# chaofengc/FeMaSR

Hardware: AMD Instinct MI355X
Metric: SR output megapixels/sec at x4 (128->512) (higher is better)
Workload: dtype f32 (1x1 convs / nn.Linear: every fp32 operand split EXACTLY into three bf16 terms, six partial products, fp32 accumulation on the bf16 matrix pipe - closer to fp64 than the fp32 fmaf chain, bit-identical to the CPU oracle)

## Files before the change

### femasr_amd/_lib.py

```python
import ctypes
import os

_HERE = os.path.dirname(os.path.abspath(__file__))
SO_PATH = os.path.join(_HERE, 'csrc', 'libfemasr_hip.so')

c_int, c_i64, c_f32 = ctypes.c_int, ctypes.c_int64, ctypes.c_float
vp, szt = ctypes.c_void_p, ctypes.c_size_t


class FemasrError(RuntimeError):
    pass


MAX_CODEBOOKS = 3


class Config(ctypes.Structure):
    _fields_ = ([(n, ctypes.c_int32) for n in ('in_channel', 'gt_resolution', 'lq_stage', 'scale_factor', 'use_quantize',
                                               'use_residual', 'n_codebooks')] +
                [(n, ctypes.c_int32 * MAX_CODEBOOKS) for n in ('codebook_scale', 'n_e', 'e_dim')] +
                [('device', ctypes.c_int32)])


class ConvArgs(ctypes.Structure):
    _fields_ = [
        ('in_', vp), ('B', ctypes.c_int32), ('H', ctypes.c_int32), ('W', ctypes.c_int32), ('Cin', ctypes.c_int32),
        ('w', vp), ('bias', vp),
        ('Cout', ctypes.c_int32), ('ksz', ctypes.c_int32), ('stride', ctypes.c_int32), ('pad', ctypes.c_int32),
        ('up2', ctypes.c_int32), ('prologue', ctypes.c_int32),
        ('pro_a', vp), ('pro_b', vp), ('pro_c', vp),
        ('act', ctypes.c_int32),
        ('res1', vp), ('res2', vp), ('out', vp),
        ('Ho', ctypes.c_int32), ('Wo', ctypes.c_int32),
        ('w_bf16x3', vp), ('gn_part', vp), ('w_up2', vp), ('w_wino', vp), ('fast_act', ctypes.c_int32), ('in_add', vp), ('w_bf16s', vp),
        ('w_f16', vp),
    ]


ABI_VERSION = 107
PRO_NONE, PRO_GN_SILU, PRO_LN = 0, 1, 2
ACT_NONE, ACT_GELU, ACT_RELU = 0, 1, 2

SIGNATURES = {
    'femasr_last_error': (ctypes.c_char_p, []),
    'femasr_version': (c_int, []),
    'femasr_create': (c_int, [ctypes.POINTER(Config), ctypes.POINTER(vp)]),
    'femasr_destroy': (None, [vp]),
    'femasr_num_weights': (c_int, [vp]),
    'femasr_weight_info': (c_int, [vp, c_int, ctypes.POINTER(ctypes.c_char_p), ctypes.POINTER(c_i64 * 4), ctypes.POINTER(c_int)]),
# ... 87 lines not shown
    'femasr_dihedral_expand': (c_int, [vp, vp, c_int, c_int, c_int, c_int, vp, vp]),
    'femasr_dihedral_expand_u8': (c_int, [vp, vp, c_int, c_int, c_int, vp, vp]),
    'femasr_dihedral_merge': (c_int, [vp, vp, vp, c_int, c_int, c_int, c_int, vp]),
    'femasr_dihedral_merge_u8': (c_int, [vp, vp, vp, c_int, c_int, c_int, vp]),
    'femasr_png_filter_rgb8': (c_int, [vp, vp, c_int, c_int, c_int, c_int, vp]),
    'femasr_clock_probe': (c_int, [vp, c_int, vp]),
    'femasr_clock_probe_entries': (c_int, []),
}
DEBUG_SIGNATURES = {
    'femasr_debug_set_wino_limits': (c_int, [vp, c_int, c_int]),
    'femasr_debug_mfma_bf16': (c_int, [vp, vp, vp, vp, c_int, vp]),
    'femasr_gemm_force_config': (c_int, [c_int]),
    'femasr_conv_small_launch_blocks': (c_int, [c_int]),
    'femasr_debug_conv_variant_name': (c_int, [ctypes.POINTER(ConvArgs), ctypes.c_char_p, c_int]),
    'femasr_debug_weight_image_bytes': (c_int, [vp, c_int, ctypes.POINTER(szt)]),
}

_lib = None


def load():
    global _lib
    if _lib is not None:
        return _lib
    if not os.path.exists(SO_PATH):
        raise FemasrError(
            f'{SO_PATH} not found: the HIP extension is not built. Run `python femasr_amd/csrc/build.py` '
            '(needs hipcc; cross-compiles gfx950 without a GPU). There is no CPU fallback.')
    lib = ctypes.CDLL(SO_PATH)
    lib.femasr_version.restype = c_int
    if lib.femasr_version() != ABI_VERSION:
# ... 19 lines not shown
```

### femasr_amd/csrc/kernels_gemm_bf16.hip

```cpp
#include "conv_common.h"
#include "detmath.h"
#include <stdlib.h>

typedef float f32x16 __attribute__((ext_vector_type(16)));
typedef __bf16 bf16x8 __attribute__((ext_vector_type(8)));
typedef __bf16 bf16x2_t __attribute__((ext_vector_type(2)));
typedef float f32x2_t __attribute__((ext_vector_type(2)));

namespace {

struct GemmSParams {
    const float *A;
    const uint4 *W;
    const float *bias, *res1, *res2;
    float *out;
    int M, N, K, MB, NB, NT32;
    int imH, imW, Cin, tapmul;
    int imHo, imWo, stride;
};

__device__ float g_gs_zero_page[64];

constexpr int GS_A_HALF = 3 * 2 * 128;
constexpr int GS_A_BYTES = 2 * GS_A_HALF * 16;
constexpr int GS_W_STAGE = 4 * 3 * 64;
constexpr int GS_W_STAGES = 4;
constexpr int GS_LDS_BYTES = GS_A_BYTES + GS_W_STAGES * GS_W_STAGE * 16;
static_assert(4 * TSCRATCH * 4 <= GS_LDS_BYTES, "epilogue scratch overlays the main-loop buffers");

__device__ __forceinline__ unsigned cvt_pk_bf16(float a, float b)
{
    const bf16x2_t r = __builtin_convertvector(f32x2_t{a, b}, bf16x2_t);
    return __builtin_bit_cast(unsigned, r);
// ... 186 lines not shown
                d1[k] = *reinterpret_cast<const f32x4_t *>(ra + o);
                if (NRES >= 2) d2[k] = *reinterpret_cast<const f32x4_t *>(rb + o);
            }
        };
        if (vec) {
#pragma unroll
            for (int j = 0; j < 2; ++j) {
                const int col = n0 + (wn * 2 + j) * 32 + 4 * tq;
                bpre[j] = *reinterpret_cast<const f32x4_t *>(p.bias + (col < p.N ? col : 0));
            }
        }
        fetch_res(0, r1[0], r2[0]);
        asm volatile("s_waitcnt lgkmcnt(0)" ::: "memory");
        __builtin_amdgcn_s_barrier();
        asm volatile("" ::: "memory");
#pragma unroll
        for (int tl = 0; tl < 4; ++tl) {
            const int i = tl >> 1, j = tl & 1;
            const int rbase = m0 + (wm * 2 + i) * 32, cbase = n0 + (wn * 2 + j) * 32;
            if (vec) {
                const int col = cbase + 4 * tq;
                const bool cok = col < p.N;
                if (tl + 1 < 4) fetch_res(tl + 1, r1[(tl + 1) & 1], r2[(tl + 1) & 1]);
#pragma unroll
                for (int r = 0; r < 16; ++r) T[((r & 3) + 8 * (r >> 2) + 4 * h) * TPITCH + c31] = hi[i][j][r] + lo[i][j][r];
                const f32x4_t b4 = bpre[j];
#pragma unroll
                for (int k = 0; k < 4; ++k) {
                    const f32x4_t a4 = *reinterpret_cast<const f32x4_t *>(T + (trow + 8 * k) * TPITCH + 4 * tq);
                    float v[4] = {a4[0] + b4[0], a4[1] + b4[1], a4[2] + b4[2], a4[3] + b4[3]};
                    if (ACT == FEMASR_ACT_GELU) {
                        const det_f32x2 g0 = det_gelu2(det_f32x2{v[0], v[1]}), g1 = det_gelu2(det_f32x2{v[2], v[3]});
                        v[0] = g0[0]; v[1] = g0[1]; v[2] = g1[0]; v[3] = g1[1];
                    }
#pragma unroll
                    for (int e = 0; e < 4; ++e) {
                        if (NRES >= 1) v[e] = v[e] + r1[tl & 1][k][e];
                        if (NRES >= 2) v[e] = v[e] + r2[tl & 1][k][e];
                    }
                    const int row = rbase + trow + 8 * k;
                    if (cok && row < p.M) *reinterpret_cast<f32x4_t *>(p.out + (size_t)row * p.N + col) = f32x4_t{v[0], v[1], v[2], v[3]};
                }
            } else {
                const int col = cbase + c31;
#pragma unroll
                for (int r = 0; r < 16; ++r) {
                    const int row = rbase + (r & 3) + 8 * (r >> 2) + 4 * h;
                    if (row < p.M && col < p.N) {
                        const size_t o = (size_t)row * p.N + col;
                        float v = (hi[i][j][r] + lo[i][j][r]) + p.bias[col];
                        if (ACT == FEMASR_ACT_GELU) v = det_gelu(v);
                        if (NRES >= 1) v = v + ra[o];
                        if (NRES >= 2) v = v + rb[o];
                        p.out[o] = v;
                    }
                }
// ... 132 lines not shown
{
    FEMASR_REQUIRE(a && a->in && w_bf16s && femasr_gemm_bf16s_shape_ok(a), "gemm_bf16s: layer is neither a 1x1 / linear layer nor a 3x3 pad-1 conv of stride 1 or 2 with Cin %% 64 == 0");
    FEMASR_REQUIRE(a->bias && a->out, "gemm_bf16s: bias/out must be set");
    FEMASR_REQUIRE(a->act == FEMASR_ACT_NONE || a->act == FEMASR_ACT_GELU, "gemm_bf16s: bad activation %d", a->act);
    const bool conv = a->ksz == 3;
    const int Ho = conv ? (a->H - 1) / a->stride + 1 : a->H, Wo = conv ? (a->W - 1) / a->stride + 1 : a->W;
    const long long M = (long long)a->B * Ho * Wo;
    FEMASR_REQUIRE(a->Ho == Ho && a->Wo == Wo, "gemm_bf16s: Ho/Wo mismatch");
    FEMASR_REQUIRE(M > 0 && M < (1ll << 31) - 256, "gemm_bf16s: bad row count");
    GemmSParams p{};
    p.A = a->in; p.W = (const uint4 *)w_bf16s; p.bias = a->bias; p.res1 = a->res1; p.res2 = a->res2; p.out = a->out;
    p.M = (int)M; p.N = a->Cout; p.K = conv ? 9 * a->Cin : a->Cin;
    p.imH = a->H; p.imW = a->W; p.imHo = Ho; p.imWo = Wo; p.stride = a->stride; p.Cin = a->Cin; p.tapmul = ((1 << 20) + (a->Cin >> 5) - 1) / (a->Cin >> 5);
    p.NT32 = (p.N + 31) / 32;
    p.MB = (p.M + 127) / 128; p.NB = (p.N + 127) / 128;
    const int vi = femasr_gemm_bf16s_pick_variant(a);
    GSVariant &v = g_gsv[vi];
    FEMASR_CHECK(femasr_allow_dynamic_lds((const void *)v.kern, &v.attr_devs, GS_LDS_BYTES));
    hipLaunchKernelGGL(v.kern, dim3((unsigned)(p.MB * p.NB)), dim3(256), (size_t)GS_LDS_BYTES, s, p);
    FEMASR_CHECK_HIP(hipGetLastError());
    if (variant_out) *variant_out = vi;
    if (flops_out) *flops_out = 2.0 * (double)M * (double)a->Cout * (double)p.K;
    return FEMASR_OK;
}
```

### femasr_amd/csrc/kernels_misc.hip

```cpp
#include "common.h"
#include "detmath.h"
#include <stdlib.h>
#include <string.h>
#include <type_traits>

namespace {

__device__ __forceinline__ float4 ld4(const float *p) { return *reinterpret_cast<const float4 *>(p); }

__device__ __forceinline__ int xcd_remap_misc(int bid, int nblk)
{
    const int q = nblk >> 3, r = nblk & 7, xcd = bid & 7, within = bid >> 3;
    return (xcd < r ? xcd * (q + 1) : r * (q + 1) + (xcd - r) * q) + within;
}

__global__ void pad_nchw_to_nhwc_kernel(const float *__restrict__ in, int B, int C, int H, int W, int Hp, int Wp,
                                        float *__restrict__ out, size_t total)
{
    for (size_t i = blockIdx.x * (size_t)blockDim.x + threadIdx.x; i < total; i += (size_t)gridDim.x * blockDim.x) {
        const int c = (int)(i % C);
        size_t r = i / C;
        const int x = (int)(r % Wp);
        r /= Wp;
        const int y = (int)(r % Hp);
// ... 287 lines not shown
    q = __builtin_fmaf(d, d, q);
    const float var = wave_tree_sum(q) * (1.0f / 256.0f);
    const float rstd = 1.0f / sqrtf(var + eps);
    const float4 g = ld4(gamma + lane * 4), b = ld4(beta + lane * 4);
    float4 o;
    o.x = __builtin_fmaf((v.x - mean) * rstd, g.x, b.x);
    o.y = __builtin_fmaf((v.y - mean) * rstd, g.y, b.y);
    o.z = __builtin_fmaf((v.z - mean) * rstd, g.z, b.z);
    o.w = __builtin_fmaf((v.w - mean) * rstd, g.w, b.w);
    *reinterpret_cast<float4 *>(y + row * 256 + lane * 4) = o;
}

constexpr int ATT_HD = 32, ATT_N = 64;
typedef float att_f32x16 __attribute__((ext_vector_type(16)));

template <int UNITS>
__global__ __launch_bounds__(64, 2) void window_attention_reg_kernel(const float *__restrict__ qkv, int B, int H, int W, int C,
                                                                     int heads, int shift, const float *__restrict__ table,
                                                                     float *__restrict__ out, int total)
{
    __shared__ float Ts[UNITS][232];
    const int lane = threadIdx.x, c = lane & 31, hf = lane >> 5;
    const int nwx = W >> 3, nwy = H >> 3;
    struct Unit { int h, wx, wy, n; };
    auto unit_of = [&](int bid) {
        Unit g;
        g.h = bid % heads;
        bid /= heads;
        g.wx = bid % nwx;
        bid /= nwx;
        g.wy = bid % nwy;
        g.n = bid / nwy;
        return g;
    };
    Unit gs[UNITS];
    bool has[UNITS];
#pragma unroll
    for (int u = 0; u < UNITS; ++u) {
        const int bid = (int)blockIdx.x * UNITS + u;
        has[u] = bid < total;
        gs[u] = unit_of(has[u] ? bid : total - 1);
        for (int i = lane; i < 225; i += 64) Ts[u][i] = table[i * heads + gs[u].h];
    }
    const float scale = 0.17677669529663687f;
    auto rowtok = [&](const Unit &g, int iy) { int y = g.wy * 8 + iy + shift; if (y >= H) y -= H; return y * W; };
    auto coltok = [&](const Unit &g, int ix) { int x = g.wx * 8 + ix + shift; if (x >= W) x -= W; return x; };
    auto qb = [&](const Unit &g) { return qkv + (size_t)g.n * H * W * 3 * C + g.h * ATT_HD; };

    float ak[2][16], bq[2][16];
    auto load_qk = [&](const Unit &g) {
        const float *qbase = qb(g);
#pragma unroll
        for (int tI = 0; tI < 2; ++tI) {
            const int w = 32 * tI + c;
            const unsigned tok = (unsigned)(rowtok(g, w >> 3) + coltok(g, w & 7));
            const float *kp = qbase + tok * (unsigned)(3 * C) + C, *qp = qbase + tok * (unsigned)(3 * C);
#pragma unroll
            for (int d4 = 0; d4 < 8; ++d4) {
                const float4 kv = ld4(kp + 4 * d4), qv = ld4(qp + 4 * d4);
                ak[tI][2 * d4] = hf ? kv.y : kv.x;
                ak[tI][2 * d4 + 1] = hf ? kv.w : kv.z;
                bq[tI][2 * d4] = (hf ? qv.y : qv.x) * scale;
                bq[tI][2 * d4 + 1] = (hf ? qv.w : qv.z) * scale;
            }
        }
    };
    load_qk(gs[0]);
#pragma unroll
    for (int u = 0; u < UNITS; ++u) {
        if (!has[u]) break;
        const Unit g = gs[u];
        const float *qbase = qb(g);
        float *obase = out + (size_t)g.n * H * W * C + g.h * ATT_HD;
        const bool masked = shift > 0 && (g.wy == nwy - 1 || g.wx == nwx - 1);
        att_f32x16 sc[2][2];
#pragma unroll
        for (int tj = 0; tj < 2; ++tj)
#pragma unroll
            for (int ti = 0; ti < 2; ++ti)
#pragma unroll
                for (int r = 0; r < 16; ++r) sc[tj][ti][r] = 0.f;
#pragma unroll
        for (int st = 0; st < 16; ++st)
#pragma unroll
            for (int tj = 0; tj < 2; ++tj)
#pragma unroll
                for (int ti = 0; ti < 2; ++ti) sc[tj][ti] = __builtin_amdgcn_mfma_f32_32x32x2f32(ak[tj][st], bq[ti][st], sc[tj][ti], 0, 0, 0);

        float vf[2][16];
        {
            const float *vb = qbase + 2 * C + c;
            unsigned cto[4];
#pragma unroll
            for (int e = 0; e < 4; ++e) cto[e] = (unsigned)coltok(g, e + 4 * hf) * (unsigned)(3 * C);
#pragma unroll
            for (int tj = 0; tj < 2; ++tj)
#pragma unroll
                for (int r = 0; r < 16; ++r) {
                    const unsigned ro = (unsigned)__builtin_amdgcn_readfirstlane(rowtok(g, (r >> 2) + 4 * tj)) * (unsigned)(3 * C);
                    vf[tj][r] = vb[ro + cto[r & 3]];
                }
        }
        if (u + 1 < UNITS && has[u + 1 < UNITS ? u + 1 : u]) load_qk(gs[u + 1 < UNITS ? u + 1 : u]);
#pragma unroll
        for (int ti = 0; ti < 2; ++ti) {
// ... 517 lines not shown
                       gamma, beta, eps, y);
    FEMASR_CHECK_HIP(hipGetLastError());
    return FEMASR_OK;
}

int femasr_window_attention(void *stream, const float *qkv, int B, int H, int W, int C, int heads, int shift,
                            const float *table, float *out)
{
    FEMASR_REQUIRE(qkv && table && out && B > 0, "window_attention: bad args");
    FEMASR_REQUIRE(H % 8 == 0 && W % 8 == 0 && H >= 8 && W >= 8, "window_attention: H,W must be multiples of 8 (%d,%d)", H, W);
    FEMASR_REQUIRE(heads > 0 && heads <= 8 && C == heads * ATT_HD, "window_attention: head_dim must be 32, at most 8 heads (C=%d heads=%d)", C, heads);
    FEMASR_REQUIRE(shift >= 0 && shift < 8, "window_attention: bad shift %d", shift);
    FEMASR_REQUIRE((size_t)H * W * 3 * C < ((size_t)1 << 30), "window_attention: image too large for 32-bit offsets");
    const size_t total = (size_t)B * (H / 8) * (W / 8) * heads;
    FEMASR_REQUIRE(total < ((size_t)1 << 31), "window_attention: too many (window, head) units");
    hipLaunchKernelGGL(window_attention_reg_kernel<1>, dim3((unsigned)total), dim3(64), 0, (hipStream_t)stream, qkv, B, H, W, C, heads, shift, table,
                       out, (int)total);
    FEMASR_CHECK_HIP(hipGetLastError());
    return FEMASR_OK;
}

int femasr_row_sqsum(void *stream, const float *x, int64_t rows, int D, float *out)
{
    FEMASR_REQUIRE(x && out && rows > 0 && D > 0 && D % 4 == 0, "row_sqsum: bad args");
    hipLaunchKernelGGL(row_sqsum_kernel, dim3((unsigned)((rows + 63) / 64)), dim3(64), 0, (hipStream_t)stream, x,
                       (long long)rows, D, out);
    FEMASR_CHECK_HIP(hipGetLastError());
    return FEMASR_OK;
}

int femasr_vq(void *stream, const float *z, int64_t M, int D, const float *cb, const float *cbT, const float *ee,
              int n_e, int64_t *idx, float *zq, void *scratch)
// ... 237 lines not shown
     offsetof(Args, w_bf16s), split_bytes, split_repack, nullptr, 1, nullptr, femasr_gemm_bf16s_shape_ok,
     "conv2d: w_bf16s given but the layer is neither a 1x1 stride-1 layer nor a 3x3 pad-1 conv of stride 1 or 2, with Cin % 64 == 0 and no prologue", nullptr},
    {CONV_F16, FORM_KERNELS(conv_f16), femasr_conv_f16_launch,
     offsetof(Args, w_f16), f16_bytes, f16_repack, femasr_repack_packed_f16, 3, not_k1, femasr_conv_f16_shape_ok,
     "conv2d: w_f16 given but the layer is not eligible for the fp16 path (the bf16x3 shape rule)", gn_tiles_mfma16},
    {CONV_GEMM_F16, FORM_KERNELS(gemm_f16), femasr_gemm_f16_launch,
     offsetof(Args, w_f16), gemm_f16_bytes, gemm_f16_repack, femasr_repack_packed_k1_f16, 3, is_k1, femasr_gemm_f16_shape_ok,
     "conv2d: w_f16 given with ksz = 1 but the layer is not a 1x1 stride-1 layer with Cin % 64 == 0 and no prologue", nullptr},
};
#undef FORM_KERNELS
const ConvFormDesc &femasr_conv_form_desc(int f) { return kConvForms[f]; }

int femasr_conv_form_launch(hipStream_t s, ConvForm f, const femasr_conv_args *a, int *slot_out, double *flops_out)
{
    int v = 0;
    const int r = kConvForms[f].launch(s, a, &v, flops_out);
    for (int g = 0; g < f; ++g) v += kConvForms[g].variant_count();
    if (slot_out) *slot_out = v;
    return r;
}

static ConvForm conv2d_form(const femasr_conv_args *a)
{
    ConvForm best = CONV_DIRECT;
    for (int f = 0; a && f < CONV_FORM_COUNT; ++f) {
        const ConvFormDesc &d = kConvForms[f];
        if (d.rank < kConvForms[best].rank && femasr_conv_form_image(f, a) && (!d.chosen || d.chosen(a))) best = (ConvForm)f;
    }
    return best;
}
// ... 24 lines not shown
```

### femasr_amd/csrc/model.hip

```cpp
#include <assert.h>
#include <stdarg.h>
#include <stdio.h>
#include <stdlib.h>
#include <string.h>

#include <algorithm>
#include <array>
#include <map>
#include <string>
#include <vector>

#include "common.h"

static thread_local char g_err[1024] = "";

int femasr_set_error(int code, const char *fmt, ...)
{
    va_list ap;
    va_start(ap, fmt);
    vsnprintf(g_err, sizeof(g_err), fmt, ap);
    va_end(ap);
    return code;
}

// ... 25 lines not shown
{
    int r = 0;
    while ((1 << (r + 1)) <= v) ++r;
    return r;
}

enum WKind { W_CONV, W_LINEAR, W_VEC, W_TABLE, W_CODEBOOK };

struct WSpec {
    std::string key;
    WKind kind;
    int64_t shape[4];
    int ndim;
    void *image[CONV_FORM_COUNT] = {};
    float *up2w = nullptr;
    float *dev() const { return (float *)image[CONV_DIRECT]; }
    int ksz() const { return kind == W_CONV ? (int)shape[2] : 1; }
    bool up2 = false;
    int stride = 1;
    bool set = false;
    size_t numel() const { size_t n = 1; for (int i = 0; i < ndim; ++i) n *= (size_t)shape[i]; return n; }
};

bool behind_every_lookup(const femasr_config &cfg, int encode_depth, int last_quant_stage, const std::string &k)
{
    const bool dec = k.rfind("decoder_group.", 0) == 0, aq = k.rfind("after_quant_group.", 0) == 0, oc = k.rfind("out_conv", 0) == 0;
    if (cfg.n_codebooks == 1) {
        if (dec || aq || oc) return true;
        const std::string pre = "multiscale_encoder.blocks.";
        return cfg.lq_stage && k.rfind(pre, 0) == 0 && atoi(k.c_str() + pre.size()) > encode_depth;
// ... 64 lines not shown
    int linear_math = FEMASR_LINEAR_MATH_BF16_SPLIT;
    int wino_log2_total = FEMASR_WINO_LOG2_TOTAL, wino_log2_image = FEMASR_WINO_LOG2_IMAGE;
};

}

struct femasr_handle {
    femasr_config cfg;
    int scale = 1, max_depth = 0, encode_depth = 0;
    int last_quant_stage = 0;
    std::vector<WSpec> specs;
    std::map<std::string, int> index;
    float *cbT[FEMASR_MAX_CODEBOOKS] = {nullptr, nullptr, nullptr}, *ee[FEMASR_MAX_CODEBOOKS] = {nullptr, nullptr, nullptr};
    void *vq_aux[FEMASR_MAX_CODEBOOKS] = {nullptr, nullptr, nullptr};
    bool finalized = false;
    unsigned decoder_seen = ((1u << FEMASR_DECODER_MATH_COUNT) - 1) & ~(1u << FEMASR_DECODER_MATH_FP16);
    unsigned linear_seen = ((1u << FEMASR_LINEAR_MATH_COUNT) - 1) & ~(1u << FEMASR_LINEAR_MATH_FP16);
    bool prof = false;
    std::vector<ProfRec> recs;
    std::vector<hipEvent_t> pool;
    size_t pool_used = 0;
    std::vector<double> acc_ms, acc_flops, acc_bytes;
    std::vector<int64_t> acc_n;
    std::vector<std::string> slot_names;
    ConvModes modes;
    int nsub = 1;
    std::vector<hipStream_t> sub_streams;
    std::vector<hipEvent_t> sub_done;
    hipEvent_t ev_fork = nullptr;
    std::map<std::array<int, 4>, std::vector<size_t>> plans;
// ... 220 lines not shown
    {
        T t; t.B = B; t.H = H; t.W = W; t.C = C;
        t.p = alloc_f(t.numel());
        return t;
    }
    void release(void *p) { if (p) arena->release(p); }
    void release(T &t) { release(t.p); t.p = nullptr; }

    struct ConvOpt {
        int ksz = 3, stride = 1, pad = 1, up2 = 0, act = 0;
        int pro = FEMASR_PRO_NONE;
        const float *pa = nullptr, *pb = nullptr, *pc = nullptr;
        const float *res1 = nullptr, *res2 = nullptr;
        const float *in_add = nullptr;
        bool want_gn = false;
    };
    femasr_conv_args conv_args(const T &x, int cout, const ConvOpt &o) const
    {
        const int Hv = o.up2 ? 2 * x.H : x.H, Wv = o.up2 ? 2 * x.W : x.W;
        femasr_conv_args a{};
        a.in = x.p; a.B = x.B; a.H = x.H; a.W = x.W; a.Cin = x.C;
        a.Cout = cout; a.ksz = o.ksz; a.stride = o.stride; a.pad = o.pad; a.up2 = o.up2;
        a.prologue = o.pro; a.pro_a = o.pa; a.pro_b = o.pb; a.pro_c = o.pc;
        a.act = o.act; a.res1 = o.res1; a.res2 = o.res2; a.in_add = o.in_add;
        a.Ho = (Hv + 2 * o.pad - o.ksz) / o.stride + 1; a.Wo = (Wv + 2 * o.pad - o.ksz) / o.stride + 1;
        return a;
    }

    T conv(const T &x, const std::string &prefix, int cout, const ConvOpt &o)
    {
        femasr_conv_args a = conv_args(x, cout, o);
        T y = alloc_t(x.B, a.Ho, a.Wo, cout);
        a.out = y.p;
        const ConvForm f = conv_form(h, h->modes, prefix, a);
        if (o.in_add && f != CONV_WINO_UP2 && !rc)
            rc = femasr_set_error(FEMASR_ERR_INVALID, "conv %s: a second input was scheduled for a conv that does not run in the x2 Winograd-type form", prefix.c_str());
        float *act_tmp = (f == CONV_SPLIT && o.pro == FEMASR_PRO_GN_SILU) ? alloc_f(x.numel()) : nullptr;
        const ConvFormDesc &form = femasr_conv_form_desc(f);
        if (o.want_gn && form.gn_tiles && (y.gn_tiles = form.gn_tiles(&a)) > 0) {
// ... 76 lines not shown
    }

    T swin_block(const T &y, int B, int H, int W, const std::string &bp, int shift)
    {
        const int rows = B * H * W, C = 256;
        auto ln = [&](const T &t, const std::string &np) {
            T o = alloc_t(1, rows, 1, C);
            if (rc || dry()) return o;
            Scope sc(h, s(), dry(), SLOT_LN, 0.0, (double)t.numel() * 8.0);
            const int r = femasr_layernorm(s(), t.p, rows, C, Wt(np + ".weight"), Wt(np + ".bias"), 1e-5f, o.p);
            if (r && !rc) rc = r;
            return o;
        };
        T n1 = ln(y, bp + ".norm1");
        ConvOpt oq; oq.ksz = 1; oq.pad = 0;
        T qkv = conv(n1, bp + ".attn.qkv", 3 * C, oq);
        release(n1);
        T att = alloc_t(1, rows, 1, C);
        if (!rc && !dry()) {
            Scope sc(h, s(), dry(), SLOT_ATTN, 4.0 * (double)rows * 64.0 * C, (double)rows * C * 16.0);
            const int r = femasr_window_attention(s(), qkv.p, B, H, W, C, 8, shift, Wt(bp + ".attn.relative_position_bias_table"), att.p);
            if (r && !rc) rc = r;
        }
        release(qkv);
        ConvOpt op; op.ksz = 1; op.pad = 0; op.res1 = y.p;
        T y1 = conv(att, bp + ".attn.proj", C, op);
        release(att);
        T n2 = ln(y1, bp + ".norm2");
        ConvOpt o1; o1.ksz = 1; o1.pad = 0; o1.act = FEMASR_ACT_GELU;
        T hdn = conv(n2, bp + ".mlp.fc1", 4 * C, o1);
        release(n2);
        ConvOpt o2; o2.ksz = 1; o2.pad = 0; o2.res1 = y1.p;
        T y2 = conv(hdn, bp + ".mlp.fc2", C, o2);
        release(hdn);
        release(y1);
        return y2;
// ... 301 lines not shown
        assert(d.form == f);
        for (int v = 0; v < d.variant_count(); ++v) h->slot_names.push_back(d.variant_name(v));
    }
    const size_t nslots = h->slot_names.size();
    h->acc_ms.assign(nslots, 0.0); h->acc_flops.assign(nslots, 0.0); h->acc_bytes.assign(nslots, 0.0); h->acc_n.assign(nslots, 0);
    *out = h;
    return FEMASR_OK;
}

void femasr_destroy(femasr_handle *h)
{
    if (!h) return;
    for (auto &w : h->specs) {
        for (void *p : w.image) if (p) (void)hipFree(p);
        if (w.up2w) (void)hipFree(w.up2w);
    }
    for (int q = 0; q < FEMASR_MAX_CODEBOOKS; ++q) {
        if (h->cbT[q]) (void)hipFree(h->cbT[q]);
        if (h->ee[q]) (void)hipFree(h->ee[q]);
        if (h->vq_aux[q]) (void)hipFree(h->vq_aux[q]);
    }
    for (auto e : h->pool) (void)hipEventDestroy(e);
    for (auto e : h->sub_done) (void)hipEventDestroy(e);
    for (auto st : h->sub_streams) (void)hipStreamDestroy(st);
    if (h->ev_fork) (void)hipEventDestroy(h->ev_fork);
    delete h;
}

int femasr_num_weights(const femasr_handle *h) { return h ? (int)h->specs.size() : 0; }

// ... 12 lines not shown
    FEMASR_REQUIRE(h && key && dev_ptr && shape, "set_weight: null argument");
    const std::string k(key);
    if (k.size() > 24 && (k.rfind(".relative_position_index") == k.size() - 24)) return FEMASR_OK;
    if (k.size() > 10 && (k.rfind(".attn_mask") == k.size() - 10)) return FEMASR_OK;
    auto it = h->index.find(k);
    if (it == h->index.end()) return femasr_set_error(FEMASR_ERR_WEIGHT, "set_weight: unknown key '%s'", key);
    DeviceGuard guard(h->cfg.device);
    FEMASR_REQUIRE(guard.ok, "set_weight: hipSetDevice(%d) failed", h->cfg.device);
    WSpec &w = h->specs[it->second];
    bool same = (ndim == w.ndim);
    for (int i = 0; same && i < ndim; ++i) same = (shape[i] == w.shape[i]);
    if (!same) return femasr_set_error(FEMASR_ERR_WEIGHT, "set_weight: shape mismatch for '%s'", key);
    if (w.kind != W_CONV && w.kind != W_LINEAR) {
        if (!w.dev()) FEMASR_CHECK_HIP(hipMalloc(&w.image[CONV_DIRECT], w.numel() * sizeof(float)));
        FEMASR_CHECK_HIP(hipMemcpyAsync(w.dev(), dev_ptr, w.numel() * sizeof(float), hipMemcpyDeviceToDevice, nullptr));
    } else {
        const int O = (int)w.shape[0], I = (int)w.shape[1];
        const std::array<bool, CONV_FORM_COUNT> can = layer_forms(h, w);
        for (int f = 0; f < CONV_FORM_COUNT; ++f) {
            if (!can[f]) continue;
            const ConvFormDesc &d = femasr_conv_form_desc(f);
            if (!w.image[f]) FEMASR_CHECK_HIP(hipMalloc(&w.image[f], d.image_bytes(O, I, w.ksz())));
            FEMASR_CHECK(d.repack(dev_ptr, O, I, w.ksz(), w.image[f]));
        }
        if (w.up2 && femasr_up2_weight_floats(O, I)) {
            if (!w.up2w) FEMASR_CHECK_HIP(hipMalloc((void **)&w.up2w, femasr_up2_weight_floats(O, I) * sizeof(float)));
            FEMASR_CHECK(femasr_repack_oihw_up2(nullptr, dev_ptr, O, I, w.up2w));
        }
    }
    FEMASR_CHECK_HIP(hipStreamSynchronize(nullptr));
// ... 226 lines not shown
    if (h->modes.decoder_math != mode) h->plans.clear();
    h->modes.decoder_math = mode;
    return FEMASR_OK;
}

int femasr_debug_set_wino_limits(femasr_handle *h, int log2_total, int log2_image)
{
    FEMASR_REQUIRE(h && log2_total >= 0 && log2_total <= FEMASR_WINO_LOG2_TOTAL && log2_image >= 0 && log2_image <= FEMASR_WINO_LOG2_IMAGE,
                   "debug_set_wino_limits: exponents are 0 (default) or up to %d / %d", FEMASR_WINO_LOG2_TOTAL, FEMASR_WINO_LOG2_IMAGE);
    h->modes.wino_log2_total = log2_total ? log2_total : FEMASR_WINO_LOG2_TOTAL;
    h->modes.wino_log2_image = log2_image ? log2_image : FEMASR_WINO_LOG2_IMAGE;
    h->plans.clear();
    return FEMASR_OK;
}

int femasr_set_linear_math(femasr_handle *h, int mode)
{
    FEMASR_REQUIRE(h && mode >= 0 && mode < FEMASR_LINEAR_MATH_COUNT, "set_linear_math: mode must be 0 (fp32 MFMA chain), 1 (bf16 three-term split) or 2 (fp16, one pass)");
    if (!(h->linear_seen >> mode & 1)) {
        h->linear_seen |= 1u << mode;
        const int rc = build_missing_images(h, "set_linear_math");
        if (rc) { h->linear_seen &= ~(1u << mode); return rc; }
    }
    if (h->modes.linear_math != mode) h->plans.clear();
    h->modes.linear_math = mode;
    return FEMASR_OK;
}

int femasr_debug_weight_image_bytes(const femasr_handle *h, int form, size_t *bytes)
{
// ... 63 lines not shown
```

### include/femasr_hip.h

```cpp
#ifndef FEMASR_HIP_H
#define FEMASR_HIP_H

#include <stddef.h>
#include <stdint.h>

#ifdef __cplusplus
extern "C" {
#endif

typedef enum {
    FEMASR_OK = 0,
    FEMASR_ERR_INVALID = -1,
    FEMASR_ERR_HIP = -2,
    FEMASR_ERR_WEIGHT = -3,
    FEMASR_ERR_WORKSPACE = -4
} femasr_status;

typedef struct femasr_handle femasr_handle;

#define FEMASR_MAX_CODEBOOKS 3
typedef struct {
    int32_t in_channel;
    int32_t gt_resolution;
    int32_t lq_stage;
// ... 60 lines not shown
    int32_t Cout, ksz, stride, pad, up2;
    int32_t prologue;
    const float *pro_a;
    const float *pro_b;
    const float *pro_c;
    int32_t act;
    const float *res1;
    const float *res2;
    float *out;
    int32_t Ho, Wo;
    const void *w_bf16x3;
    double *gn_part;
    const float *w_up2;
    const float *w_wino;
    int32_t fast_act;
    const float *in_add;
    const void *w_bf16s;
    const void *w_f16;
} femasr_conv_args;
int femasr_conv2d(void *stream, const femasr_conv_args *a);

size_t femasr_gn_scratch_bytes(int B, int H, int W, int C, int G);
int femasr_gn_coeffs(void *stream, const float *x, int B, int H, int W, int C, int G,
                     const float *gamma, const float *beta, float eps, float *a, float *b, void *scratch);
int femasr_gn_coeffs_from_partials(void *stream, const double *part, int B, int tiles, int H, int W, int C, int G,
                                   const float *gamma, const float *beta, float eps, float *a, float *b);
int femasr_gn_silu_apply(void *stream, const float *x, int B, int H, int W, int C, const float *a, const float *b, float *y);
int femasr_ln_stats(void *stream, const float *x, int64_t rows, int C, float eps, float *stats);
int femasr_layernorm(void *stream, const float *x, int64_t rows, int C, const float *gamma, const float *beta,
                     float eps, float *y);
int femasr_window_attention(void *stream, const float *qkv, int B, int H, int W, int C, int heads, int shift,
                            const float *table, float *out);
int femasr_vq(void *stream, const float *z, int64_t M, int D, const float *cb, const float *cbT,
              const float *ee, int n_e, int64_t *idx, float *zq, void *scratch);
// ... 105 lines not shown
```

### include/femasr_hip_debug.h

```cpp
#ifndef FEMASR_HIP_DEBUG_H
#define FEMASR_HIP_DEBUG_H
#include "femasr_hip.h"
#ifdef __cplusplus
extern "C" {
#endif

int femasr_debug_set_wino_limits(femasr_handle *h, int log2_total, int log2_image);

int femasr_debug_mfma_bf16(void *stream, const uint16_t *a, const uint16_t *b, const float *c, int n, float *d);

int femasr_gemm_force_config(int cfg);
int femasr_conv_small_launch_blocks(int blocks);

int femasr_debug_conv_variant_name(const femasr_conv_args *a, char *name, int cap);

int femasr_debug_weight_image_bytes(const femasr_handle *h, int form, size_t *bytes);

#ifdef __cplusplus
}
#endif
#endif
```

Measured before the change: 67.64.

## Write QKV projection directly in window-major layout for window attention

The split-bf16 1x1 GEMM epilogue for the attention qkv projection can now scatter its output straight into a per-(window, head) contiguous layout, with the cyclic shift folded in. A new window-attention kernel variant reads Q, K and V from contiguous 6144-float blocks instead of gathering shifted rows across the raster image. The relative-position bias table is also pre-packed per head. The aim is fewer strided, poorly coalesced reads in attention, at the cost of more address arithmetic and scattered stores in the GEMM epilogue, plus a change to the ABI struct layout.

```diff
diff --git a/femasr_amd/_lib.py b/femasr_amd/_lib.py
--- a/femasr_amd/_lib.py
+++ b/femasr_amd/_lib.py
@@ -32,7 +32,8 @@
         ('act', ctypes.c_int32),
         ('res1', vp), ('res2', vp), ('out', vp),
         ('Ho', ctypes.c_int32), ('Wo', ctypes.c_int32),
-        ('w_bf16x3', vp), ('gn_part', vp), ('w_up2', vp), ('w_wino', vp), ('fast_act', ctypes.c_int32), ('in_add', vp), ('w_bf16s', vp),
+        ('w_bf16x3', vp), ('gn_part', vp), ('w_up2', vp), ('w_wino', vp), ('fast_act', ctypes.c_int32), ('out_order', ctypes.c_int32),
+        ('in_add', vp), ('w_bf16s', vp),
         ('w_f16', vp),
     ]
 
@@ -150,7 +151,14 @@
     'femasr_conv_small_launch_blocks': (c_int, [c_int]),
     'femasr_debug_conv_variant_name': (c_int, [ctypes.POINTER(ConvArgs), ctypes.c_char_p, c_int]),
     'femasr_debug_weight_image_bytes': (c_int, [vp, c_int, ctypes.POINTER(szt)]),
+    'femasr_pack_bias_table': (c_int, [vp, vp, c_int, vp]),
+    'femasr_window_attention_wm': (c_int, [vp, vp, c_int, c_int, c_int, c_int, c_int, c_int, vp, vp]),
+    'femasr_debug_set_raster_qkv': (c_int, [vp, c_int]),
 }
+
+
+def out_order_windows(h, w, shift):
+    return 1 | (shift << 1) | ((w >> 3) << 4) | ((h >> 3) << 17)
 
 _lib = None
 
diff --git a/femasr_amd/csrc/kernels_gemm_bf16.hip b/femasr_amd/csrc/kernels_gemm_bf16.hip
--- a/femasr_amd/csrc/kernels_gemm_bf16.hip
+++ b/femasr_amd/csrc/kernels_gemm_bf16.hip
@@ -17,6 +17,8 @@
     int M, N, K, MB, NB, NT32;
     int imH, imW, Cin, tapmul;
     int imHo, imWo, stride;
+    int order, oH, oW, oshift, oC;
+    unsigned hw_mul, hw_sh, w_mul, w_sh;
 };
 
 __device__ float g_gs_zero_page[64];
@@ -233,6 +235,29 @@
         asm volatile("s_waitcnt lgkmcnt(0)" ::: "memory");
         __builtin_amdgcn_s_barrier();
         asm volatile("" ::: "memory");
+        const bool wmo = ACT == FEMASR_ACT_NONE && NRES == 0 && CONV == 0 && p.order;
+        long long w_s[2][4] = {};
+        unsigned w_l[2][4] = {};
+        if (wmo) {
+            const int cb0 = n0 + wn * 64, which = (cb0 >= p.oC ? 1 : 0) + (cb0 >= 2 * p.oC ? 1 : 0);
+            const unsigned wU = (unsigned)p.oC * 192u;
+            const unsigned wmul = which < 2 ? 4u : 32u;
+            const unsigned pre = which < 2 ? (unsigned)tq * 256u : 4u * (unsigned)tq;
+#pragma unroll
+            for (int i = 0; i < 2; ++i)
+#pragma unroll
+                for (int k = 0; k < 4; ++k) {
+                    const unsigned rg = (unsigned)(m0 + (wm * 2 + i) * 32 + 8 * k);
+                    const unsigned n = __umulhi(rg, p.hw_mul) >> p.hw_sh, rem = rg - n * (unsigned)(p.oH * p.oW);
+                    const unsigned y = __umulhi(rem, p.w_mul) >> p.w_sh, x0 = rem - y * (unsigned)p.oW;
+                    int yy = (int)y - p.oshift, xx = (int)x0 + trow - p.oshift;
+                    yy = yy < 0 ? yy + p.oH : yy;
+                    xx = xx < 0 ? xx + p.oW : xx;
+                    w_s[i][k] = (long long)n * ((long long)p.oH * p.oW * p.N) + (long long)((unsigned)((yy >> 3) * (p.oW >> 3)) * wU + (unsigned)(8 * (yy & 7)) * wmul) +
+                                (long long)(which * 2048 - which * p.oC * 192);
+                    w_l[i][k] = (unsigned)(xx >> 3) * wU + (unsigned)(xx & 7) * wmul + pre;
+                }
+        }
 #pragma unroll
         for (int tl = 0; tl < 4; ++tl) {
             const int i = tl >> 1, j = tl & 1;
@@ -258,7 +283,12 @@
                         if (NRES >= 2) v[e] = v[e] + r2[tl & 1][k][e];
                     }
                     const int row = rbase + trow + 8 * k;
-                    if (cok && row < p.M) *reinterpret_cast<f32x4_t *>(p.out + (size_t)row * p.N + col) = f32x4_t{v[0], v[1], v[2], v[3]};
+                    if (wmo) {
+                        float *base = p.out + (w_s[i][k] + (long long)((cbase >> 5) * 6144));
+                        if (cok && row < p.M) *reinterpret_cast<f32x4_t *>(base + w_l[i][k]) = f32x4_t{v[0], v[1], v[2], v[3]};
+                    } else {
+                        if (cok && row < p.M) *reinterpret_cast<f32x4_t *>(p.out + (size_t)row * p.N + col) = f32x4_t{v[0], v[1], v[2], v[3]};
+                    }
                 }
             } else {
                 const int col = cbase + c31;
@@ -421,6 +451,21 @@
     p.imH = a->H; p.imW = a->W; p.imHo = Ho; p.imWo = Wo; p.stride = a->stride; p.Cin = a->Cin; p.tapmul = ((1 << 20) + (a->Cin >> 5) - 1) / (a->Cin >> 5);
     p.NT32 = (p.N + 31) / 32;
     p.MB = (p.M + 127) / 128; p.NB = (p.N + 127) / 128;
+    if (a->out_order) {
+        const int o = a->out_order, oH = ((o >> 17) & 0x1fff) * 8, oW = ((o >> 4) & 0x1fff) * 8, shift = (o >> 1) & 7;
+        FEMASR_REQUIRE((o & 1) && o > 0 && oH > 0 && oW > 0, "gemm_bf16s: bad out_order 0x%x", o);
+        FEMASR_REQUIRE(!conv && !a->res1 && !a->res2 && a->act == FEMASR_ACT_NONE, "gemm_bf16s: out_order is taken by a plain 1x1 layer only");
+        FEMASR_REQUIRE(p.N % 192 == 0 && M % ((long long)oH * oW) == 0, "gemm_bf16s: out_order needs Cout = 3 C with C %% 64 == 0 and whole %d x %d images (Cout=%d rows=%lld)", oH, oW, p.N, M);
+        auto magic = [](unsigned d, unsigned &mul, unsigned &sh) {
+            unsigned l = 0;
+            while ((1ull << l) < d) ++l;
+            const unsigned long long m = (1ull << (31 + l)) / d + 1;
+            mul = (unsigned)m; sh = l - 1;
+            return m <= 0xffffffffull;
+        };
+        FEMASR_REQUIRE((long long)oH * oW * p.N < (1ll << 30) && magic((unsigned)(oH * oW), p.hw_mul, p.hw_sh) && magic((unsigned)oW, p.w_mul, p.w_sh), "gemm_bf16s: out_order image too large");
+        p.order = 1; p.oH = oH; p.oW = oW; p.oshift = shift; p.oC = p.N / 3;
+    }
     const int vi = femasr_gemm_bf16s_pick_variant(a);
     GSVariant &v = g_gsv[vi];
     FEMASR_CHECK(femasr_allow_dynamic_lds((const void *)v.kern, &v.attr_devs, GS_LDS_BYTES));
diff --git a/femasr_amd/csrc/kernels_misc.hip b/femasr_amd/csrc/kernels_misc.hip
--- a/femasr_amd/csrc/kernels_misc.hip
+++ b/femasr_amd/csrc/kernels_misc.hip
@@ -325,7 +325,7 @@
 constexpr int ATT_HD = 32, ATT_N = 64;
 typedef float att_f32x16 __attribute__((ext_vector_type(16)));
 
-template <int UNITS>
+template <int UNITS, bool WM>
 __global__ __launch_bounds__(64, 2) void window_attention_reg_kernel(const float *__restrict__ qkv, int B, int H, int W, int C,
                                                                      int heads, int shift, const float *__restrict__ table,
                                                                      float *__restrict__ out, int total)
@@ -351,24 +351,26 @@
         const int bid = (int)blockIdx.x * UNITS + u;
         has[u] = bid < total;
         gs[u] = unit_of(has[u] ? bid : total - 1);
-        for (int i = lane; i < 225; i += 64) Ts[u][i] = table[i * heads + gs[u].h];
+        for (int i = lane; i < 225; i += 64) Ts[u][i] = WM ? table[gs[u].h * 232 + i] : table[i * heads + gs[u].h];
     }
     const float scale = 0.17677669529663687f;
     auto rowtok = [&](const Unit &g, int iy) { int y = g.wy * 8 + iy + shift; if (y >= H) y -= H; return y * W; };
     auto coltok = [&](const Unit &g, int ix) { int x = g.wx * 8 + ix + shift; if (x >= W) x -= W; return x; };
     auto qb = [&](const Unit &g) { return qkv + (size_t)g.n * H * W * 3 * C + g.h * ATT_HD; };
+    auto ub = [&](const Unit &g) { return qkv + (size_t)(((g.n * nwy + g.wy) * nwx + g.wx) * heads + g.h) * 6144; };
 
     float ak[2][16], bq[2][16];
     auto load_qk = [&](const Unit &g) {
-        const float *qbase = qb(g);
+        const float *qbase = WM ? ub(g) : qb(g);
 #pragma unroll
         for (int tI = 0; tI < 2; ++tI) {
             const int w = 32 * tI + c;
-            const unsigned tok = (unsigned)(rowtok(g, w >> 3) + coltok(g, w & 7));
-            const float *kp = qbase + tok * (unsigned)(3 * C) + C, *qp = qbase + tok * (unsigned)(3 * C);
+            const unsigned tok = WM ? 0u : (unsigned)(rowtok(g, w >> 3) + coltok(g, w & 7));
+            const float *kp = WM ? qbase + 2048 + 4 * w : qbase + tok * (unsigned)(3 * C) + C, *qp = WM ? qbase + 4 * w : qbase + tok * (unsigned)(3 * C);
+            constexpr int dstep = WM ? 256 : 4;
 #pragma unroll
             for (int d4 = 0; d4 < 8; ++d4) {
-                const float4 kv = ld4(kp + 4 * d4), qv = ld4(qp + 4 * d4);
+                const float4 kv = ld4(kp + dstep * d4), qv = ld4(qp + dstep * d4);
                 ak[tI][2 * d4] = hf ? kv.y : kv.x;
                 ak[tI][2 * d4 + 1] = hf ? kv.w : kv.z;
                 bq[tI][2 * d4] = (hf ? qv.y : qv.x) * scale;
@@ -381,7 +383,7 @@
     for (int u = 0; u < UNITS; ++u) {
         if (!has[u]) break;
         const Unit g = gs[u];
-        const float *qbase = qb(g);
+        const float *qbase = WM ? ub(g) : qb(g);
         float *obase = out + (size_t)g.n * H * W * C + g.h * ATT_HD;
         const bool masked = shift > 0 && (g.wy == nwy - 1 || g.wx == nwx - 1);
         att_f32x16 sc[2][2];
@@ -399,7 +401,13 @@
                 for (int ti = 0; ti < 2; ++ti) sc[tj][ti] = __builtin_amdgcn_mfma_f32_32x32x2f32(ak[tj][st], bq[ti][st], sc[tj][ti], 0, 0, 0);
 
         float vf[2][16];
-        {
+        if (WM) {
+            const float *vb = qbase + 4096 + c;
+#pragma unroll
+            for (int tj = 0; tj < 2; ++tj)
+#pragma unroll
+                for (int r = 0; r < 16; ++r) vf[tj][r] = vb[((r & 3) + 8 * (r >> 2) + 4 * hf + 32 * tj) * 32];
+        } else {
             const float *vb = qbase + 2 * C + c;
             unsigned cto[4];
 #pragma unroll
@@ -947,8 +955,40 @@
     FEMASR_REQUIRE((size_t)H * W * 3 * C < ((size_t)1 << 30), "window_attention: image too large for 32-bit offsets");
     const size_t total = (size_t)B * (H / 8) * (W / 8) * heads;
     FEMASR_REQUIRE(total < ((size_t)1 << 31), "window_attention: too many (window, head) units");
-    hipLaunchKernelGGL(window_attention_reg_kernel<1>, dim3((unsigned)total), dim3(64), 0, (hipStream_t)stream, qkv, B, H, W, C, heads, shift, table,
+    hipLaunchKernelGGL((window_attention_reg_kernel<1, false>), dim3((unsigned)total), dim3(64), 0, (hipStream_t)stream, qkv, B, H, W, C, heads, shift, table,
                        out, (int)total);
+    FEMASR_CHECK_HIP(hipGetLastError());
+    return FEMASR_OK;
+}
+
+int femasr_window_attention_wm(void *stream, const float *qkv_wm, int B, int H, int W, int C, int heads, int shift,
+                               const float *table_packed, float *out)
+{
+    FEMASR_REQUIRE(qkv_wm && table_packed && out && B > 0, "window_attention_wm: bad args");
+    FEMASR_REQUIRE(H % 8 == 0 && W % 8 == 0 && H >= 8 && W >= 8, "window_attention_wm: H,W must be multiples of 8 (%d,%d)", H, W);
+    FEMASR_REQUIRE(heads > 0 && heads <= 8 && C == heads * ATT_HD, "window_attention_wm: head_dim must be 32, at most 8 heads (C=%d heads=%d)", C, heads);
+    FEMASR_REQUIRE(shift >= 0 && shift < 8, "window_attention_wm: bad shift %d", shift);
+    FEMASR_REQUIRE((size_t)H * W * 3 * C < ((size_t)1 << 30), "window_attention_wm: image too large for 32-bit offsets");
+    const size_t total = (size_t)B * (H / 8) * (W / 8) * heads;
+    FEMASR_REQUIRE(total < ((size_t)1 << 31), "window_attention_wm: too many (window, head) units");
+    hipLaunchKernelGGL((window_attention_reg_kernel<1, true>), dim3((unsigned)total), dim3(64), 0, (hipStream_t)stream, qkv_wm, B, H, W, C, heads, shift,
+                       table_packed, out, (int)total);
+    FEMASR_CHECK_HIP(hipGetLastError());
+    return FEMASR_OK;
+}
+
+__global__ void pack_bias_table_kernel(const float *__restrict__ table, int heads, float *__restrict__ out)
+{
+    const int i = blockIdx.x * blockDim.x + threadIdx.x;
+    if (i >= heads * 232) return;
+    const int h = i / 232, e = i - h * 232;
+    out[i] = e < 225 ? table[e * heads + h] : 0.f;
+}
+
+int femasr_pack_bias_table(void *stream, const float *table, int heads, float *out)
+{
+    FEMASR_REQUIRE(table && out && heads > 0 && heads <= 8, "pack_bias_table: bad args");
+    hipLaunchKernelGGL(pack_bias_table_kernel, dim3((unsigned)((heads * 232 + 255) / 256)), dim3(256), 0, (hipStream_t)stream, table, heads, out);
     FEMASR_CHECK_HIP(hipGetLastError());
     return FEMASR_OK;
 }
@@ -1216,6 +1256,7 @@
 int femasr_conv_form_launch(hipStream_t s, ConvForm f, const femasr_conv_args *a, int *slot_out, double *flops_out)
 {
     int v = 0;
+    FEMASR_REQUIRE(!a->out_order || f == CONV_SPLIT, "conv: out_order is only taken by the split-bf16 form of a 1x1 layer (w_bf16s)");
     const int r = kConvForms[f].launch(s, a, &v, flops_out);
     for (int g = 0; g < f; ++g) v += kConvForms[g].variant_count();
     if (slot_out) *slot_out = v;
diff --git a/femasr_amd/csrc/model.hip b/femasr_amd/csrc/model.hip
--- a/femasr_amd/csrc/model.hip
+++ b/femasr_amd/csrc/model.hip
@@ -63,6 +63,7 @@
     int ndim;
     void *image[CONV_FORM_COUNT] = {};
     float *up2w = nullptr;
+    float *table_t = nullptr;
     float *dev() const { return (float *)image[CONV_DIRECT]; }
     int ksz() const { return kind == W_CONV ? (int)shape[2] : 1; }
     bool up2 = false;
@@ -157,6 +158,7 @@
     float *cbT[FEMASR_MAX_CODEBOOKS] = {nullptr, nullptr, nullptr}, *ee[FEMASR_MAX_CODEBOOKS] = {nullptr, nullptr, nullptr};
     void *vq_aux[FEMASR_MAX_CODEBOOKS] = {nullptr, nullptr, nullptr};
     bool finalized = false;
+    bool raster_qkv = false;
     unsigned decoder_seen = ((1u << FEMASR_DECODER_MATH_COUNT) - 1) & ~(1u << FEMASR_DECODER_MATH_FP16);
     unsigned linear_seen = ((1u << FEMASR_LINEAR_MATH_COUNT) - 1) & ~(1u << FEMASR_LINEAR_MATH_FP16);
     bool prof = false;
@@ -407,6 +409,7 @@
         const float *res1 = nullptr, *res2 = nullptr;
         const float *in_add = nullptr;
         bool want_gn = false;
+        int out_order = 0;
     };
     femasr_conv_args conv_args(const T &x, int cout, const ConvOpt &o) const
     {
@@ -415,7 +418,7 @@
         a.in = x.p; a.B = x.B; a.H = x.H; a.W = x.W; a.Cin = x.C;
         a.Cout = cout; a.ksz = o.ksz; a.stride = o.stride; a.pad = o.pad; a.up2 = o.up2;
         a.prologue = o.pro; a.pro_a = o.pa; a.pro_b = o.pb; a.pro_c = o.pc;
-        a.act = o.act; a.res1 = o.res1; a.res2 = o.res2; a.in_add = o.in_add;
+        a.act = o.act; a.res1 = o.res1; a.res2 = o.res2; a.in_add = o.in_add; a.out_order = o.out_order;
         a.Ho = (Hv + 2 * o.pad - o.ksz) / o.stride + 1; a.Wo = (Wv + 2 * o.pad - o.ksz) / o.stride + 1;
         return a;
     }
@@ -522,12 +525,16 @@
         };
         T n1 = ln(y, bp + ".norm1");
         ConvOpt oq; oq.ksz = 1; oq.pad = 0;
+        const bool wm = !h->raster_qkv && conv_form(h, h->modes, bp + ".attn.qkv", conv_args(n1, 3 * C, oq)) == CONV_SPLIT;
+        if (wm) oq.out_order = FEMASR_OUT_ORDER_WINDOWS(H, W, shift);
         T qkv = conv(n1, bp + ".attn.qkv", 3 * C, oq);
         release(n1);
         T att = alloc_t(1, rows, 1, C);
         if (!rc && !dry()) {
             Scope sc(h, s(), dry(), SLOT_ATTN, 4.0 * (double)rows * 64.0 * C, (double)rows * C * 16.0);
-            const int r = femasr_window_attention(s(), qkv.p, B, H, W, C, 8, shift, Wt(bp + ".attn.relative_position_bias_table"), att.p);
+            const WSpec *tb = spec(bp + ".attn.relative_position_bias_table");
+            const int r = !tb ? rc : wm ? femasr_window_attention_wm(s(), qkv.p, B, H, W, C, 8, shift, tb->table_t, att.p)
+                                        : femasr_window_attention(s(), qkv.p, B, H, W, C, 8, shift, tb->dev(), att.p);
             if (r && !rc) rc = r;
         }
         release(qkv);
@@ -859,6 +866,7 @@
     for (auto &w : h->specs) {
         for (void *p : w.image) if (p) (void)hipFree(p);
         if (w.up2w) (void)hipFree(w.up2w);
+        if (w.table_t) (void)hipFree(w.table_t);
     }
     for (int q = 0; q < FEMASR_MAX_CODEBOOKS; ++q) {
         if (h->cbT[q]) (void)hipFree(h->cbT[q]);
@@ -901,6 +909,11 @@
     if (w.kind != W_CONV && w.kind != W_LINEAR) {
         if (!w.dev()) FEMASR_CHECK_HIP(hipMalloc(&w.image[CONV_DIRECT], w.numel() * sizeof(float)));
         FEMASR_CHECK_HIP(hipMemcpyAsync(w.dev(), dev_ptr, w.numel() * sizeof(float), hipMemcpyDeviceToDevice, nullptr));
+        if (w.kind == W_TABLE) {
+            const int heads = (int)w.shape[1];
+            if (!w.table_t) FEMASR_CHECK_HIP(hipMalloc((void **)&w.table_t, (size_t)heads * 232 * sizeof(float)));
+            FEMASR_CHECK(femasr_pack_bias_table(nullptr, w.dev(), heads, w.table_t));
+        }
     } else {
         const int O = (int)w.shape[0], I = (int)w.shape[1];
         const std::array<bool, CONV_FORM_COUNT> can = layer_forms(h, w);
@@ -1157,6 +1170,13 @@
     return FEMASR_OK;
 }
 
+int femasr_debug_set_raster_qkv(femasr_handle *h, int on)
+{
+    FEMASR_REQUIRE(h, "debug_set_raster_qkv: null handle");
+    h->raster_qkv = on != 0;
+    return FEMASR_OK;
+}
+
 int femasr_set_linear_math(femasr_handle *h, int mode)
 {
     FEMASR_REQUIRE(h && mode >= 0 && mode < FEMASR_LINEAR_MATH_COUNT, "set_linear_math: mode must be 0 (fp32 MFMA chain), 1 (bf16 three-term split) or 2 (fp16, one pass)");
diff --git a/include/femasr_hip.h b/include/femasr_hip.h
--- a/include/femasr_hip.h
+++ b/include/femasr_hip.h
@@ -98,10 +98,12 @@
     const float *w_up2;
     const float *w_wino;
     int32_t fast_act;
+    int32_t out_order;
     const float *in_add;
     const void *w_bf16s;
     const void *w_f16;
 } femasr_conv_args;
+#define FEMASR_OUT_ORDER_WINDOWS(H, W, shift) (1 | ((shift) << 1) | (((W) >> 3) << 4) | (((H) >> 3) << 17))
 int femasr_conv2d(void *stream, const femasr_conv_args *a);
 
 size_t femasr_gn_scratch_bytes(int B, int H, int W, int C, int G);
diff --git a/include/femasr_hip_debug.h b/include/femasr_hip_debug.h
--- a/include/femasr_hip_debug.h
+++ b/include/femasr_hip_debug.h
@@ -16,6 +16,11 @@
 
 int femasr_debug_weight_image_bytes(const femasr_handle *h, int form, size_t *bytes);
 
+int femasr_pack_bias_table(void *stream, const float *table, int heads, float *out);
+int femasr_window_attention_wm(void *stream, const float *qkv_wm, int B, int H, int W, int C, int heads, int shift,
+                               const float *table_packed, float *out);
+int femasr_debug_set_raster_qkv(femasr_handle *h, int on);
+
 #ifdef __cplusplus
 }
 #endif
```

Result: no change. 67.80, median of 6 (+0.2%).
